# sakarias88/racer-tracer

Measured on AMD Instinct MI355X. Metric: Msamples/s (W*H*spp/s) at 1920x1080, higher is better.
Workload: dtype f64; 1 GPU; cornell_box.yml 1920x1080 1024spp max_depth 20; strip_rows=8, parallelism=image rows interleaved over 1 GPU(s)

## Files before the change

### racer-tracer_amd/csrc/rt_pool_coop.h

```cpp
#pragma once
#include "rt_pool_groups.h"
#include "rt_pool_lds.h"
#include "rt_primary_bounds.h"

namespace RT_KNS {

__device__ __forceinline__ int lane_rank(uint64_t mask) {
    return (int)__builtin_amdgcn_mbcnt_hi((uint32_t)(mask >> 32), __builtin_amdgcn_mbcnt_lo((uint32_t)mask, 0u));
}

__device__ __forceinline__ void post_request(SphereSlot *slot, const ScatterPrefix &P, uint32_t base) {
    __hip_atomic_store(&slot->b, P.b, __ATOMIC_RELAXED, __HIP_MEMORY_SCOPE_WAVEFRONT);
    __hip_atomic_store(&slot->y, P.y, __ATOMIC_RELAXED, __HIP_MEMORY_SCOPE_WAVEFRONT);
    __hip_atomic_store(&slot->x, P.x, __ATOMIC_RELAXED, __HIP_MEMORY_SCOPE_WAVEFRONT);
    __hip_atomic_store(&slot->w, P.w, __ATOMIC_RELAXED, __HIP_MEMORY_SCOPE_WAVEFRONT);
    __hip_atomic_store(&slot->z, P.z, __ATOMIC_RELAXED, __HIP_MEMORY_SCOPE_WAVEFRONT);
    __hip_atomic_store(&slot->base, base, __ATOMIC_RELAXED, __HIP_MEMORY_SCOPE_WAVEFRONT);
}
__device__ __forceinline__ void move_masked(const d3 &p, uint64_t mask, d3 &v) {
    uint64_t saved;
    asm volatile("s_and_saveexec_b64 %[saved], %[mask]\n\t"
                 "v_mov_b64 %[x], %[px]\n\t"
                 "v_mov_b64 %[y], %[py]\n\t"
                 "v_mov_b64 %[z], %[pz]\n\t"
                 "s_mov_b64 exec, %[saved]"
                 : [x] "+v"(v.x), [y] "+v"(v.y), [z] "+v"(v.z), [saved] "=&s"(saved)
                 : [mask] "s"(mask), [px] "v"(p.x), [py] "v"(p.y), [pz] "v"(p.z)
                 : "scc");
}
__device__ __forceinline__ void increment_masked(uint32_t &v, uint64_t mask) {
    asm("v_addc_co_u32 %[v], vcc, 0, %[v], %[mask]" : [v] "+v"(v) : [mask] "s"(mask) : "vcc");
}
static_assert(sizeof(TraceArgs) % alignof(rtdev::PrimaryRects) == 0, "no padding between the kernel's two arguments");
__device__ __forceinline__ const RT_CONSTANT rtdev::PrimaryRects *primary_rects_here() {
    return (const RT_CONSTANT rtdev::PrimaryRects *)((const RT_CONSTANT unsigned char *)kernargs_here() + sizeof(TraceArgs));
}
__device__ __forceinline__ uint32_t request_count(uint64_t pending) {
    uint32_t n = (uint32_t)__builtin_popcountll(pending);
    asm("" : "+s"(n));
    return n;
}

static_assert(rtdev::RT_PRIMARY_RECTS <= 32, "a rect mask is one 32-bit word");
template <bool PAIRS>
__device__ __forceinline__ void closest_hit_rects(const Prim *table, const d3 &o, const d3 &d, const d3 &inv_d, double &best_t, int &best,
                                                  uint32_t rect_mask = ~0u) {
    auto test_plane = [&](auto axis, const Prim &P, int i) {
#ifndef RT_EXACT_DIV
        rect_closest_update<decltype(axis)::value>(P.p[0], P.p[1], P.p[2], P.p[3], P.p[4], o, d, inv_d, 0.001, best_t, best, i);
        return;
#endif
        double t;
        if (rect_t<true>(decltype(axis)::value, P.p[0], P.p[1], P.p[2], P.p[3], P.p[4], o, d, inv_d, 0.001, best_t, t)) {
            best_t = t;
            best = i;
        }
    };
    const Prim *rec = table;
    int i = 0;
    auto group = [&](auto axis, int end) {
        if (PAIRS) {
            for (; i + 1 < end; i += 2, rec += 2) {
                const Prim pa = load_prim_uniform(rec, 0), pb = load_prim_uniform(rec, 1);
                test_plane(axis, pa, i);
                test_plane(axis, pb, i + 1);
            }
            if (i < end) {
                test_plane(axis, load_prim_uniform(rec, 0), i);
                ++i;
                ++rec;
            }
        } else {
            const int n = end - i;
            if (n > 0 && n < 32 && ((rect_mask >> (i & 31)) & ((1u << n) - 1u)) == 0u) {
                i = end;
                rec = reinterpret_cast<const Prim *>(reinterpret_cast<const unsigned char *>(rec) + (uint32_t)n * (uint32_t)sizeof(Prim));
            }
            for (; i < end; ++i, ++rec)
                if ((rect_mask >> (i & 31)) & 1u) test_plane(axis, load_prim_uniform(rec, 0), i);
        }
    };
    const RT_CONSTANT TraceArgs *KB = kernargs_here();
    const int end_xy = KB->rect_end[0], end_xz = KB->rect_end[1], end_yz = KB->rect_end[2];
    group(std::integral_constant<int, 2>(), end_xy);
    group(std::integral_constant<int, 1>(), end_xz);
    group(std::integral_constant<int, 0>(), end_yz);
}

template <int MAX_ROUNDS>
__device__ __forceinline__ uint64_t coop_random_in_unit_sphere(uint64_t pending, uint32_t pixel, uint32_t sample, uint32_t seg,
                                                           uint32_t &base, uint32_t k0, uint32_t k1, int lane,
                                                           SphereSlot *slot, d3 &result) {
    uint64_t have = 0;
    const ScatterPrefix own = scatter_prefix(pixel, sample, seg, k0, k1);
    auto one_round = [&](int round) {
        const bool FIRST = round == 0;
        const uint32_t n = request_count(pending);
        if (!FIRST && n < 8u) return false;
        const int lg = rt_groups::group_lg(n);
        d3 cand;
        uint64_t take;
        if (lg == 0) {
            const d3 p = sphere_candidate(philox_from_prefix(own, base, k0, k1));
            cand = p;
            take = pending;
            const uint64_t inside = ballot(len2(p) < 1.0);
            have |= pending & inside;
            pending &= ~inside;
            if (__builtin_amdgcn_inverse_ballot_w64(pending)) base += 1u;
        } else {
            const rt_groups::GroupMasks groups = rt_groups::group_masks((uint32_t)lg);
            const bool need = __builtin_amdgcn_inverse_ballot_w64(pending);
            const int rank = lane_rank(pending);
            if (need) post_request(slot + rank, own, base);
            const int j = lane >> lg;
            const int c = lane & ((1 << lg) - 1);
            const bool serving = (uint32_t)j < n;
            SphereSlot *const served = slot + (serving ? j : 0);
            const ScatterPrefix r = {served->b, served->y, served->x, served->w, served->z};
            const uint32_t i = served->base + (uint32_t)c;
            const d3 p = sphere_candidate(philox_from_prefix(r, i, k0, k1));
            const uint64_t accepted = ballot(serving) & ballot(len2(p) < 1.0);
            asm volatile("" ::: "memory");
            if (__builtin_amdgcn_inverse_ballot_w64(rt_groups::lowest_in_groups(accepted, groups))) {
                double *const answer = reinterpret_cast<double *>(served);
                answer[0] = p.x;
                answer[1] = p.y;
                answer[2] = p.z;
            }
            asm volatile("" ::: "memory");
            const int first = need ? (rank << lg) : 0;
            const uint64_t got = pending & ballot(((accepted >> first) & groups.width) != 0);
            const double *const answer = reinterpret_cast<const double *>(slot + (need ? rank : 0));
            cand = mk(answer[0], answer[1], answer[2]);
            take = got;
            have |= got;
            pending &= ~got;
            if (__builtin_amdgcn_inverse_ballot_w64(pending)) base += 1u << lg;
        }
        if (FIRST) {
            result = cand;
        } else {
            move_masked(cand, take, result);
        }
        return true;
    };
    if constexpr (MAX_ROUNDS == 2) {
#pragma unroll
// ... 100 lines not shown
```

### racer-tracer_amd/csrc/rt_scene_create.hip

```cpp
#include <hip/hip_runtime.h>
#include <stdint.h>
#include <string.h>
#include <memory>
#include <mutex>
#include <string>
#include <vector>
#include "rt_scene.h"

using rtapi::DevBuf;
using rtapi::fail;

namespace {
struct CachedSet {
    int device;
    rtapi::RenderBuffers buf;
};
std::mutex g_cache_mutex;
std::vector<CachedSet> g_cache;
const size_t kCachedSetsPerDevice = 2;

void render_cache_put(RtScene *s) {
    if (s->buf.complete()) {
        std::lock_guard<std::mutex> lock(g_cache_mutex);
        size_t held = 0;
        for (const CachedSet &c : g_cache) held += c.device == s->device;
        if (held < kCachedSetsPerDevice) {
            g_cache.push_back(CachedSet{s->device, s->buf});
            s->buf = rtapi::RenderBuffers();
            return;
        }
    }
    s->buf.free_all(s->device);
}
bool render_cache_take(RtScene *s) {
    std::lock_guard<std::mutex> lock(g_cache_mutex);
    int best = -1;
    for (size_t i = 0; i < g_cache.size(); ++i)
        if (g_cache[i].device == s->device && (best < 0 || g_cache[i].buf.partial.count > g_cache[(size_t)best].buf.partial.count))
            best = (int)i;
    if (best < 0) return false;
    s->buf = g_cache[(size_t)best].buf;
    g_cache.erase(g_cache.begin() + best);
    return true;
}

#define RT_FAST_LAUNCHER(member, name, ret, params) name,
#define RT_EXACT_LAUNCHER(member, name, ret, params) name##_exact,
const rtapi::Launchers kFastLaunchers = {RT_LAUNCHER_LIST(RT_FAST_LAUNCHER)};
const rtapi::Launchers kExactLaunchers = {RT_LAUNCHER_LIST(RT_EXACT_LAUNCHER)};
#undef RT_FAST_LAUNCHER
#undef RT_EXACT_LAUNCHER

template <class T> int upload(DevBuf<T> &buf, const std::vector<T> &host) {
    RT_HIP(buf.alloc(host.size()));
    if (!host.empty()) RT_HIP(hipMemcpy(buf.ptr, host.data(), host.size() * sizeof(T), hipMemcpyHostToDevice));
    return RT_OK;
}

int upload_images(const RtSceneDesc *d, RtScene *s, std::vector<rtdev::Image> &images) {
    images.assign((size_t)d->n_images, rtdev::Image());
    s->image_pixels.assign((size_t)d->n_images, nullptr);
    for (int i = 0; i < d->n_images; ++i) {
        size_t bytes = (size_t)d->images[i].width * (size_t)d->images[i].height * 4;
        RT_HIP(hipMalloc((void **)&s->image_pixels[(size_t)i], bytes));
        RT_HIP(hipMemcpy(s->image_pixels[(size_t)i], d->images[i].rgba, bytes, hipMemcpyHostToDevice));
        images[(size_t)i].rgba = s->image_pixels[(size_t)i];
        images[(size_t)i].width = d->images[i].width;
        images[(size_t)i].height = d->images[i].height;
    }
    return RT_OK;
}

rtdev::BvhBuild choose_bvh(const RtSceneDesc *d, const RtScene *s) {
    using rtapi::kBvhLdsBytes;
    auto blocks_with = [&](const rtdev::BvhBuild &b) {
        const size_t bytes = b.nodes.size() * sizeof(rtdev::BvhNode);
        const size_t dyn = rtdev::pool_lds_layout(true, s->textured, d->n_primitives, d->n_textures, bytes <= kBvhLdsBytes ? (int)b.nodes.size() : 0,
                                                  d->n_perlins > 0 && s->perlin_identity, false, s->has_moving).bytes;
        return s->kernels->pool_blocks_per_cu(s->prims_class, s->textured, s->specular, 1, dyn);
    };
    const bool surely_large = d->n_primitives > 2048;
    rtdev::BvhBuild bvh = rtdev::build_bvh(d->primitives, d->n_primitives, 4, surely_large);
    int max_leaf = 0;
#ifdef RT_DEVELOPER_KNOBS
    if (const char *k = getenv("RT_BVH_LEAF")) max_leaf = atoi(k);
#endif
    if (max_leaf > 0) {
        bvh = rtdev::build_bvh(d->primitives, d->n_primitives, max_leaf);
    } else if (bvh.nodes.size() * sizeof(rtdev::BvhNode) <= kBvhLdsBytes) {
// ... 45 lines not shown
        s->pool_dyn_lds = dyn_lds(false);
        s->pool_dyn_lds_lens = dyn_lds(true);
        s->pool_static_lds = s->kernels->pool_static_lds(s->prims_class, s->textured, s->specular, s->use_bvh);
        if (s->pool_static_lds < 0) return fail(RT_ERR_HIP, "hipFuncGetAttributes of the trace kernel failed");
        s->pool_blocks_per_cu = s->kernels->pool_blocks_per_cu(s->prims_class, s->textured, s->specular, s->use_bvh, s->pool_dyn_lds);
        s->pool_blocks_per_cu_lens = s->kernels->pool_blocks_per_cu(s->prims_class, s->textured, s->specular, s->use_bvh, s->pool_dyn_lds_lens);
    }
#ifdef RT_DEVELOPER_KNOBS
    if (const char *k = getenv("RT_POOL_BLOCKS_PER_CU"))
        if (atoi(k) > 0) s->pool_blocks_per_cu = s->pool_blocks_per_cu_lens = atoi(k);
#endif
    return RT_OK;
}

int acquire_render_buffers(RtScene *s) {
    rtapi::RenderBuffers &b = s->buf;
    if (!render_cache_take(s)) {
        RT_HIP(b.segments.alloc(rtdev::RT_STAT_SLOTS));
        RT_HIP(hipStreamCreateWithFlags(&b.stream, hipStreamNonBlocking));
        RT_HIP(hipEventCreate(&b.ev_begin));
        RT_HIP(hipEventCreate(&b.ev_traced));
        RT_HIP(hipEventCreate(&b.ev_resolved));
        RT_HIP(hipHostMalloc((void **)&b.host_flags, (rtdev::RT_MAX_REGIONS + 1) * sizeof(unsigned int),
                             hipHostMallocPortable | hipHostMallocMapped | hipHostMallocCoherent));
        memset(b.host_flags, 0, (rtdev::RT_MAX_REGIONS + 1) * sizeof(unsigned int));
        RT_HIP(hipStreamCreateWithFlags(&b.stream_ctl, hipStreamNonBlocking));
    }
    RT_HIP(hipMemsetAsync(b.segments.ptr, 0, rtdev::RT_STAT_SLOTS * sizeof(unsigned long long), b.stream));
    return RT_OK;
}

int scene_create(const RtSceneDesc *d, int device, const RtSceneOptions *options, RtScene **out) {
    if (!out) return fail(RT_ERR_INVALID_ARGUMENT, "out is NULL");
    *out = nullptr;
    int rc = rtapi::validate_desc(d);
    if (rc != RT_OK) return rc;
    RtSceneOptions opt;
    if ((rc = rtapi::check_options(options, opt)) != RT_OK) return rc;
    int n_dev = rt_device_count();
    if (n_dev <= 0) return fail(RT_ERR_NO_DEVICE, "no HIP device is visible to this process");
    if (device < 0 || device >= n_dev) return fail(RT_ERR_INVALID_ARGUMENT, "device index out of range");
    RT_HIP(hipSetDevice(device));

    RtScene *s = new RtScene();
    std::unique_ptr<RtScene, void (*)(RtScene *)> half_built(s, rt_scene_destroy);
    s->device = device;
    s->exact = opt.arithmetic == RT_ARITH_REFERENCE;
    s->gather_staged = opt.gather == RT_GATHER_STAGED;
    s->use_v1 = opt.kernel == RT_KERNEL_V1;

    std::vector<rtdev::Prim> prims = rtapi::pack_prims(d);
    s->radiance_bound = rtapi::scene_radiance_bound(d);
    const std::vector<rtdev::Perlin> perlins = rtapi::pack_perlins(d, s->perlin_identity);
    const rtapi::Selection sel = rtapi::select_variant(d);
    s->prims_class = sel.prims_class;
    s->textured = sel.textured;
    s->specular = sel.specular;
    s->has_moving = sel.has_moving;
    rtapi::scene_bounds(d, s->box_mn, s->box_mx);
    s->use_bvh = d->n_primitives > rtapi::kBvhThreshold;
    if (opt.closest_hit != RT_HIT_AUTO) s->use_bvh = opt.closest_hit == RT_HIT_BVH && d->n_primitives > 0;
    if (s->radiance_bound == 0.0 && !s->use_v1 && (s->use_bvh || s->prims_class == 2)) s->exact = true;
    s->kernels = s->exact ? &kExactLaunchers : &kFastLaunchers;
    if (!s->use_bvh && (size_t)d->n_primitives * sizeof(rtdev::Prim) > rtapi::kLinearTableBytes)
        return fail(RT_ERR_UNSUPPORTED, "RT_HIT_LINEAR: the primitive table does not fit in LDS");

    std::vector<int32_t> order((size_t)d->n_primitives);
    for (size_t j = 0; j < order.size(); ++j) order[j] = (int32_t)j;
    rtdev::BvhBuild bvh;
    rtapi::LeafTable leaves;
    if (s->use_bvh) {
        bvh = choose_bvh(d, s);
        order.assign(bvh.prim_index.begin(), bvh.prim_index.end());
        std::vector<rtdev::Prim> ordered(prims.size());
        for (size_t j = 0; j < bvh.prim_index.size(); ++j) ordered[j] = prims[(size_t)bvh.prim_index[j]];
        prims.swap(ordered);
        leaves = rtapi::leaf_geometry(prims);
    } else {
        const rtapi::LinearGroups groups = rtapi::group_linear_table(prims, order);
        for (int g = 0; g < 3; ++g) s->rect_end[g] = groups.rect_end[g];
        s->sphere_end = groups.sphere_end;
        s->box_end = groups.box_end;
        const int n_rects = groups.rect_end[2];
        if (n_rects == d->n_primitives && n_rects <= rtdev::RT_PRIMARY_RECTS)
            for (int j = 0; j < n_rects; ++j) {
                const rtdev::Prim &q = prims[(size_t)j];
                s->primary_rect_geo.push_back(rtdev::RectGeo{j < groups.rect_end[0] ? 2 : (j < groups.rect_end[1] ? 1 : 0), q.p[0], q.p[1], q.p[2], q.p[3], q.p[4]});
            }
    }
    const rtapi::LightTables lights = rtapi::light_tables(d, order, rtapi::kMaxLights);

    std::vector<rtdev::Image> images;
    if ((rc = upload_images(d, s, images)) != RT_OK) return rc;
    const std::vector<rtdev::Texture> textures = rtapi::pack_textures(d, images);
    if (s->use_bvh && (rc = upload_bvh(s, bvh, leaves)) != RT_OK) return rc;
    if ((rc = rtapi::build_light_list(s, lights)) != RT_OK) return rc;
    s->light_facts = rtapi::light_facts(d);
    s->table_order = order;
    s->pick_weights.assign(lights.lights.size(), lights.lights.empty() ? 0.0 : 1.0 / (double)lights.lights.size());
    if ((rc = upload(s->prims, prims)) != RT_OK) return rc;
    if ((rc = upload(s->textures, textures)) != RT_OK) return rc;
    if ((rc = upload(s->images, images)) != RT_OK) return rc;
    if ((rc = upload(s->perlins, perlins)) != RT_OK) return rc;
    s->n_prims = d->n_primitives;
    s->n_materials = d->n_materials;
    s->n_textures = d->n_textures;
    s->n_images = d->n_images;
    s->n_perlins = d->n_perlins;
    s->bg.kind = d->background.kind;
    for (int k = 0; k < 3; ++k) {
        s->bg.top[k] = d->background.top[k];
        s->bg.bottom[k] = d->background.bottom[k];
    }
    if ((rc = size_pool(s)) != RT_OK) return rc;
    if ((rc = acquire_render_buffers(s)) != RT_OK) return rc;
    *out = half_built.release();
    return RT_OK;
}

}

extern "C" {

void rt_scene_destroy(RtScene *s) {
    if (!s) return;
    (void)hipSetDevice(s->device);
    if (s->buf.stream) (void)hipStreamSynchronize(s->buf.stream);
    if (s->buf.stream_ctl) (void)hipStreamSynchronize(s->buf.stream_ctl);
    for (uint8_t *p : s->image_pixels)
        if (p) (void)hipFree(p);
    s->prims.release();
    s->textures.release();
    s->images.release();
    s->perlins.release();
    s->bvh_nodes.release();
    s->bvh_nodes_ordered.release();
    s->bvh_prim_index.release();
    s->leaf_geo.release();
    s->nee_slot.release();
    s->nee_prim.release();
    s->nee_pick.release();
    if (rtapi::guarded("rt_scene_destroy", [&] { render_cache_put(s); return RT_OK; }) != RT_OK) s->buf.free_all(s->device);
    delete s;
}

void rt_release_cached_buffers(void) {
    (void)rtapi::guarded("rt_release_cached_buffers", [] {
        std::vector<CachedSet> all;
        {
            std::lock_guard<std::mutex> lock(g_cache_mutex);
            all.swap(g_cache);
        }
        for (CachedSet &c : all) c.buf.free_all(c.device);
        return RT_OK;
    });
}

int rt_scene_create(const RtSceneDesc *d, int device, RtScene **out) {
    return rtapi::guarded("rt_scene_create", [&] { return scene_create(d, device, nullptr, out); });
}

int rt_scene_create_ex(const RtSceneDesc *d, int device, const RtSceneOptions *options, RtScene **out) {
    return rtapi::guarded("rt_scene_create_ex", [&] { return scene_create(d, device, options, out); });
}

int rtdev_scene_classify(const RtSceneDesc *d, int32_t out[4]) {
// ... 37 lines not shown
```

### racer-tracer_amd/csrc/rt_trace_common.h

```cpp
#pragma once
#include <hip/hip_runtime.h>
#include <stdint.h>
#include "rt_device_types.h"
#include "rt_bvh_slab.h"
#include "../../include/rt_abi.h"
#include "../../include/rt_rng.h"

#ifdef RT_EXACT_DIV
#define RT_KNS rtdev_exact
#define RT_LAUNCHER(name) name##_exact
#else
#define RT_KNS rtdev_fast
#define RT_LAUNCHER(name) name
#endif

namespace RT_KNS {
using namespace rtdev;

#define RT_CONSTANT __attribute__((address_space(4)))
__device__ __forceinline__ Prim load_prim_uniform(const Prim *table, int i) {
    Prim p;
    __builtin_memcpy(&p, (const RT_CONSTANT Prim *)(table + i), sizeof(Prim));
    return p;
}
// ... 152 lines not shown
    const uint32_t d_hi = __builtin_amdgcn_alignbit(0x400u, w, 12);
    return __longlong_as_double((long long)(((unsigned long long)d_hi << 32) | d_lo)) - 3.0;
}
__device__ __forceinline__ double sym42(uint32_t w, uint32_t t_at_10) {
    return sym42_bits((w << 20) | t_at_10, w);
}
__device__ __forceinline__ d3 sphere_candidate(const u4 &b) {
    return mk(sym42_bits(__builtin_amdgcn_alignbit(b.a, b.d << 22, 12), b.a), sym42(b.b, b.d & 0x000FFC00u),
              sym42(b.c, (b.d >> 10) & 0x000FFC00u));
}

struct PathRng {
    uint32_t pixel, sample, k0, k1;
    __device__ __forceinline__ u4 block(uint32_t segment, uint32_t purpose, uint32_t blk) const {
        return philox4x32(pixel, sample, (segment << 8) | purpose, blk, k0, k1);
    }
};

__device__ __forceinline__ d3 random_in_unit_sphere(const PathRng &rng, uint32_t segment) {
    for (uint32_t i = 0;; ++i) {
        d3 p = sphere_candidate(rng.block(segment, RT_RNG_SCATTER, i));
        if (len2(p) >= 1.0) continue;
        return p;
    }
}

struct Hit {
    d3 point, normal;
    double u, v;
    bool front;
    bool uv_approx;
};

__device__ __forceinline__ void set_face_normal(Hit &h, d3 dir, d3 outward) {
    h.front = dot(dir, outward) < 0.0;
    const uint32_t flip = h.front ? 0u : 0x80000000u;
    auto with_sign = [flip](double x) {
        return __longlong_as_double((long long)((unsigned long long)__double_as_longlong(x) ^ ((unsigned long long)flip << 32)));
    };
    h.normal = mk(with_sign(outward.x), with_sign(outward.y), with_sign(outward.z));
}

__device__ __forceinline__ void set_face_normal_axis(Hit &h, d3 dir, int axis) {
#ifdef RT_EXACT_DIV
    set_face_normal(h, dir, mk(axis == 0 ? 1.0 : 0.0, axis == 1 ? 1.0 : 0.0, axis == 2 ? 1.0 : 0.0));
#else
    auto against = [](double dk) {
        const uint32_t hi = 0xBFF00000u ^ ((uint32_t)((unsigned long long)__double_as_longlong(dk) >> 32) & 0x80000000u);
        return __longlong_as_double((long long)((unsigned long long)hi << 32));
    };
    h.normal = mk(axis == 0 ? against(dir.x) : 0.0, axis == 1 ? against(dir.y) : 0.0, axis == 2 ? against(dir.z) : 0.0);
    h.front = h.normal.x + h.normal.y + h.normal.z > 0.0;
#endif
}

__device__ __forceinline__ d3 rot_fwd(d3 a, double s, double c) {
    return mk(c * a.x - s * a.z, a.y, s * a.x + c * a.z);
}
__device__ __forceinline__ d3 rot_back(d3 a, double s, double c) {
    return mk(c * a.x + s * a.z, a.y, -s * a.x + c * a.z);
}

template <bool EARLY_OUT>
__device__ __forceinline__ bool rect_t(int axis, double a0, double a1, double b0, double b1, double k,
                                       d3 o, d3 d, d3 inv_d, double t_min, double t_max, double &t_out) {
    int ia = axis == 0 ? 1 : 0;
    int ib = axis == 2 ? 1 : 2;
    const double t = div_by(k - comp(o, axis), comp(d, axis), comp(inv_d, axis));
    if (EARLY_OUT) {
        if (t < t_min || t > t_max) return false;
        const double a = comp(o, ia) + t * comp(d, ia);
        const double b = comp(o, ib) + t * comp(d, ib);
        if (a < a0 || a > a1 || b < b0 || b > b1) return false;
        t_out = t;
        return true;
    }
    const double a = comp(o, ia) + t * comp(d, ia);
    const double b = comp(o, ib) + t * comp(d, ib);
    const bool miss = (t < t_min) | (t > t_max) | (a < a0) | (a > a1) | (b < b0) | (b > b1);
    t_out = t;
    return !miss;
}

template <int AXIS>
__device__ __forceinline__ void rect_closest_update(double a0, double a1, double b0, double b1, double k, d3 o, d3 d, d3 inv_d,
                                                    double t_min, double &best_t, int &best, int i) {
    constexpr int IA = AXIS == 0 ? 1 : 0, IB = AXIS == 2 ? 1 : 2;
    double t, a, b;
    unsigned long long saved;
    asm volatile("v_add_f64 %[t], %[k], -%[oc]\n\t"
                 "v_mul_f64 %[t], %[inv], %[t]\n\t"
                 "s_mov_b64 %[saved], exec\n\t"
                 "v_cmpx_ngt_f64 %[tmin], %[t]\n\t"
                 "v_cmpx_ngt_f64 %[t], %[bt]\n\t"
                 "s_cbranch_execz 1f\n\t"
                 "v_fma_f64 %[a], %[da], %[t], %[oa]\n\t"
                 "v_fma_f64 %[b], %[db], %[t], %[ob]\n\t"
                 "v_cmpx_ngt_f64 %[a0], %[a]\n\t"
                 "v_cmpx_nlt_f64 %[a1], %[a]\n\t"
                 "v_cmpx_ngt_f64 %[b0], %[b]\n\t"
                 "v_cmpx_nlt_f64 %[b1], %[b]\n\t"
                 "v_mov_b64 %[bt], %[t]\n\t"
                 "v_mov_b32 %[best], %[i]\n"
                 "1:\n\t"
                 "s_mov_b64 exec, %[saved]"
                 : [t] "=&v"(t), [a] "=&v"(a), [b] "=&v"(b), [saved] "=&s"(saved), [bt] "+v"(best_t), [best] "+v"(best)
                 : [k] "s"(k), [oc] "v"(comp(o, AXIS)), [inv] "v"(comp(inv_d, AXIS)), [tmin] "s"(t_min), [da] "v"(comp(d, IA)),
                   [oa] "v"(comp(o, IA)), [db] "v"(comp(d, IB)), [ob] "v"(comp(o, IB)), [a0] "s"(a0), [a1] "s"(a1), [b0] "s"(b0),
                   [b1] "s"(b1), [i] "s"(i)
                 : "vcc");
}

__device__ __forceinline__ void box_side(const double *p, int s, int &axis, double &a0, double &a1,
                                         double &b0, double &b1, double &k) {
    axis = 2 - (s >> 1);
    if (axis == 2) { a0 = p[0]; a1 = p[3]; b0 = p[1]; b1 = p[4]; k = (s & 1) ? p[2] : p[5]; }
    else if (axis == 1) { a0 = p[0]; a1 = p[3]; b0 = p[2]; b1 = p[5]; k = (s & 1) ? p[1] : p[4]; }
    else { a0 = p[1]; a1 = p[4]; b0 = p[2]; b1 = p[5]; k = (s & 1) ? p[0] : p[3]; }
}

__device__ __forceinline__ bool sphere_t(d3 center, double radius2, d3 o, d3 d, double inv_a, double t_min, double t_max,
                                         double &t_out) {
    const d3 oc = o - center;
    const double a = len2(d);
    const double half_b = dot(oc, d);
    const double c = len2(oc) - radius2;
    const double disc = half_b * half_b - a * c;
    if (disc < 0.0) return false;
    const double sqrtd = sqrt_fast(disc);
    double root = div_by(-half_b - sqrtd, a, inv_a);
    if (root < t_min || t_max < root) {
        root = div_by(-half_b + sqrtd, a, inv_a);
        if (root < t_min || t_max < root) return false;
    }
    t_out = root;
    return true;
}

__device__ __forceinline__ bool box_slab_t(const double *p, d3 o, d3 d, d3 inv_d, double t_min, double t_max, double &t_out,
                                           int &side) {
    const double x_mn = div_by(p[0] - o.x, d.x, inv_d.x), x_mx = div_by(p[3] - o.x, d.x, inv_d.x);
    const double y_mn = div_by(p[1] - o.y, d.y, inv_d.y), y_mx = div_by(p[4] - o.y, d.y, inv_d.y);
    const double z_mn = div_by(p[2] - o.z, d.z, inv_d.z), z_mx = div_by(p[5] - o.z, d.z, inv_d.z);
    const double x_near = fmin(x_mn, x_mx), x_far = fmax(x_mn, x_mx);
    const double y_near = fmin(y_mn, y_mx), y_far = fmax(y_mn, y_mx);
    const double z_near = fmin(z_mn, z_mx), z_far = fmax(z_mn, z_mx);
    const double t_enter = fmax(fmax(x_near, y_near), z_near);
    const double t_exit = fmin(fmin(x_far, y_far), z_far);
    const bool entry = t_enter >= t_min;
    const double t = entry ? t_enter : t_exit;
    const int side_in = t_enter == z_near ? 0 : (t_enter == y_near ? 2 : 4);
    const int side_out = t_exit == z_far ? 0 : (t_exit == y_far ? 2 : 4);
    side = entry ? side_in : side_out;
    t_out = t;
    return t_enter <= t_exit && t >= t_min && t <= t_max;
}

template <int PRIMS>
__device__ __forceinline__ bool prim_t(const Prim &P, d3 o, d3 d, d3 inv_d, double inv_a, double time, double t_min,
                                       double t_max, double &t_out, int &aux) {
    aux = 0;
    if (PRIMS == PRIMS_RECTS) {
        int kind = P.kind;
        if (kind == RT_PRIM_XY_RECT) return rect_t<true>(2, P.p[0], P.p[1], P.p[2], P.p[3], P.p[4], o, d, inv_d, t_min, t_max, t_out);
        if (kind == RT_PRIM_XZ_RECT) return rect_t<true>(1, P.p[0], P.p[1], P.p[2], P.p[3], P.p[4], o, d, inv_d, t_min, t_max, t_out);
        return rect_t<true>(0, P.p[0], P.p[1], P.p[2], P.p[3], P.p[4], o, d, inv_d, t_min, t_max, t_out);
    }
    if (PRIMS == PRIMS_ANY) {
        if (P.flags & RT_PRIM_HAS_TRANSLATE) o = o - ld3(P.tr);
        if (P.flags & RT_PRIM_HAS_ROTATE_Y) {
            o = rot_fwd(o, P.rot_sin, P.rot_cos);
            d = rot_fwd(d, P.rot_sin, P.rot_cos);
            inv_d.x = rcp_f64(d.x);
            inv_d.z = rcp_f64(d.z);
        }
    }
    switch (PRIMS == PRIMS_SPHERES ? (int)RT_PRIM_SPHERE : P.kind) {
    case RT_PRIM_MOVING_SPHERE:
    case RT_PRIM_SPHERE: {
        d3 center = ld3(P.p);
        if (PRIMS == PRIMS_ANY && P.kind == RT_PRIM_MOVING_SPHERE)
            center = center + ((time - P.rot_sin) * P.rot_cos) * ld3(P.tr);
        return sphere_t(center, P.radius2, o, d, inv_a, t_min, t_max, t_out);
    }
    case RT_PRIM_XY_RECT: return rect_t<true>(2, P.p[0], P.p[1], P.p[2], P.p[3], P.p[4], o, d, inv_d, t_min, t_max, t_out);
    case RT_PRIM_XZ_RECT: return rect_t<true>(1, P.p[0], P.p[1], P.p[2], P.p[3], P.p[4], o, d, inv_d, t_min, t_max, t_out);
    case RT_PRIM_YZ_RECT: return rect_t<true>(0, P.p[0], P.p[1], P.p[2], P.p[3], P.p[4], o, d, inv_d, t_min, t_max, t_out);
    default: {
#ifndef RT_EXACT_DIV
        return box_slab_t(P.p, o, d, inv_d, t_min, t_max, t_out, aux);
#endif
        bool any = false;
        double closest = t_max;
// ... 409 lines not shown
```

### racer-tracer_amd/csrc/rt_trace_pool_kernel.hip

```cpp
#include <cstddef>
#include <type_traits>
#include "rt_trace_common.h"
#include "rt_primary_bounds.h"
#include "rt_variant_dispatch.h"
#include "rt_pool_profile.h"
#include "rt_pool_lds.h"
#include "rt_pool_coop.h"
#include "rt_pool_deliver.h"

#ifndef RT_OCC_TEX
#define RT_OCC_TEX 4
#endif
#ifndef RT_OCC_TEX_BVH
#define RT_OCC_TEX_BVH 4
#endif
#ifndef RT_OCC_TEX_ANY
#define RT_OCC_TEX_ANY 4
#endif
#ifndef RT_OCC_SPEC
#define RT_OCC_SPEC 5
#endif
#ifndef RT_OCC_ANY
#define RT_OCC_ANY 5
#endif
// ... 492 lines not shown
                        d = mk(signed_like(0u), signed_like(1u), signed_like(2u));
                        T = mk(1.0, 1.0, 1.0);
                        seg = 0;
                        asm volatile("; hand_out_end");
                    }
                    alive_m |= taking;
                }
                RT_REGION(2);
                if (alive_m == 0) break;
                uint64_t ended_m = 0;
                const uint64_t hit_m = alive_m & ~waiting_m;
                int kind;
                asm volatile("" : "=v"(kind));
                if (__builtin_amdgcn_inverse_ballot_w64(hit_m)) {
                    const Prim &P = lds_prims[best];
                    const Material &M = P.mat;
                    kind = M.kind;
                    RT_REGION(8);
                    T = T * ld3(M.color);
                    RT_REGION(9);
                    cand_base = 0;
#ifndef RT_EXACT_DIV
                    {
                        const int axis = P.kind == RT_PRIM_XY_RECT ? 2 : (P.kind == RT_PRIM_XZ_RECT ? 1 : 0);
                        auto against = [](double dk, bool on_axis) {
                            uint32_t lo = 0u;
                            asm volatile("" : "+v"(lo));
                            const uint32_t hi = on_axis ? 0xBFF00000u ^ ((uint32_t)((unsigned long long)__double_as_longlong(dk) >> 32) & 0x80000000u) : 0u;
                            return __longlong_as_double((long long)((unsigned long long)hi << 32 | lo));
                        };
                        const uint64_t xy_m = ballot(axis == 2), xz_m = ballot(axis == 1);
                        d = mk(against(d.x, __builtin_amdgcn_inverse_ballot_w64(~(xy_m | xz_m))), against(d.y, __builtin_amdgcn_inverse_ballot_w64(xz_m)),
                               against(d.z, __builtin_amdgcn_inverse_ballot_w64(xy_m)));
                    }
#else
                    {
                        Hit h;
                        set_face_normal_axis(h, d, P.kind == RT_PRIM_XY_RECT ? 2 : (P.kind == RT_PRIM_XZ_RECT ? 1 : 0));
                        d = h.normal;
                    }
#endif
                }
                asm volatile("" : "+v"(kind));
                const uint64_t light_m = hit_m & ballot(kind == RT_MAT_DIFFUSE_LIGHT);
                ended_m |= light_m;
                waiting_m |= hit_m & ~light_m;
                RT_REGION(4);
                d3 sph = mk(0.0, 0.0, 0.0);
                const uint64_t finish_m = coop_random_in_unit_sphere<2>(waiting_m, rng.pixel, rng.sample, seg, cand_base, A.seed_lo, A.seed_hi, lane,
                                                                        L.scratch.sphere, sph);
                waiting_m &= ~finish_m;
                RT_REGION(5);
                if (__builtin_amdgcn_inverse_ballot_w64(finish_m)) {
                    const d3 dir = d + unit_fast(sph);
                    const uint64_t near_zero = ballot(fabs(dir.x) < 1e-8) & ballot(fabs(dir.y) < 1e-8) & ballot(fabs(dir.z) < 1e-8);
#ifndef RT_EXACT_DIV
                    d = dir;
                    if (near_zero != 0) {
                        asm volatile("; near_zero (keeps the compiler from turning the branch back into selects)");
                        if ((near_zero >> lane) & 1ull) {
                            const d3 u = unit_fast(sph);
                            d = mk(rint(-u.x) + 0.0, rint(-u.y) + 0.0, rint(-u.z) + 0.0);
                        }
                    }
#else
                    const d3 normal = d;
                    d = dir;
                    if (near_zero != 0) {
                        asm volatile("; near_zero (keeps the compiler from turning the branch back into selects)");
                        if ((near_zero >> lane) & 1ull) d = normal;
                    }
#endif
                }
                increment_masked(seg, finish_m);
                const uint64_t deep_m = finish_m & ballot((int)seg >= A.max_depth);
                ended_m |= deep_m;
                const uint64_t shooting = finish_m & ~deep_m;
                RT_LANES(__popcll(shooting), next >= total);
                asm volatile("" : "=v"(best));
                if (__builtin_amdgcn_inverse_ballot_w64(shooting)) {
                    double best_t = __builtin_inf();
                    best = -1;
                    ++n_segments;
                    closest_hit_rects<true>(A.prims, o, d, rcp3(d), best_t, best);
                    asm volatile("; hit_point_begin" : "+v"(best_t));
                    o = ray_at(o, best_t, d);
                    asm volatile("; hit_point_end" : "+v"(o.x), "+v"(o.y), "+v"(o.z));
                    RT_REGION(3);
                }
                const uint64_t miss_m = shooting & ballot(best < 0);
                uint64_t adding_m = ended_m;
                ended_m |= miss_m;
                if (kernargs_here()->bg_black == 0) {
                    adding_m = ended_m;
                    const RT_CONSTANT TraceArgs *K = kernargs_here();
                    const uint64_t sky_m = K->bg.kind == RT_BG_SKY ? miss_m : 0ull;
                    if (__builtin_amdgcn_inverse_ballot_w64(miss_m & ~sky_m)) {
                        T.x = T.x * K->bg.top[0];
                        T.y = T.y * K->bg.top[1];
                        T.z = T.z * K->bg.top[2];
                    }
                    if (__builtin_amdgcn_inverse_ballot_w64(sky_m)) {
                        const double t = 0.5 * (unit_fast(d).y + 1.0);
                        T = T * ((1.0 - t) * ld3(K->bg.top) + t * ld3(K->bg.bottom));
                    }
                }
                if (__builtin_amdgcn_inverse_ballot_w64(adding_m)) {
                    atomicAdd(&L.sum[spix][0], T.x);
                    atomicAdd(&L.sum[spix][1], T.y);
                    atomicAdd(&L.sum[spix][2], T.z);
                }
                alive_m &= ~ended_m;
                RT_REGION(6);
            }
        } else
        for (;;) {
        while (next >= batch_due) {
            prepare_batch(batches_done++);
            batch_due = batches_done >= n_batches ? ~0u : (batches_done < (uint32_t)NBUF ? 0u : (batches_done - (uint32_t)(NBUF - 1)) << 6);
        }
        RT_REGION(1);
        if (next < total) {
            const uint64_t idle = ~alive_m;
            const uint32_t w = next + (uint32_t)lane_rank(idle);
            const uint32_t ready = NBUF == 2 ? total : min(total, batches_done << 6);
            next = min(next + (uint32_t)__popcll(idle), ready);
            if (OVERLAP && next >= total) state |= POOL_DRY;
            int s_off, pix_new;
            if (n_valid == 64) {
                pix_new = (int)(w & 63u);
                s_off = (int)(w >> 6);
            } else {
                s_off = (int)(w / (uint32_t)n_valid);
                pix_new = L.pix_of[w - (uint32_t)s_off * (uint32_t)n_valid];
            }
            const uint32_t pixel_new = (uint32_t)shfl_i((int)my_pixel, pix_new);
            const uint64_t taking = idle & ballot(w < ready);
            if (__builtin_amdgcn_inverse_ballot_w64(taking)) {
                spix = (int)(state & CUR) | pix_new;
                rng.pixel = pixel_new;
                rng.sample = (uint32_t)(smp0 + s_off);
                const RT_CONSTANT TraceArgs *K = kernargs_here();
                const int buf = (int)((w >> 6) & (uint32_t)(NBUF - 1)), slot = (int)(w & 63u);
                const double v = L.v[buf][slot];
                const d3 co = ld3(K->cam.origin);
                o = co;
                if (OVERLAP) d = (ld3(L.ulc) + L.u[pix_new] * ld3(K->cam.horizontal)) - v * ld3(K->cam.vertical) - co;
                else d = ld3(L.base[pix_new]) - v * ld3(K->cam.vertical) - co;
                const double lr = K->cam.lens_radius;
                if (lr != 0.0) {
                    const d3 offset = ld3(K->cam.right) * lens[buf][slot][0] + ld3(K->cam.up) * lens[buf][slot][1];
                    o = co + offset;
                    d = d - offset;
                }
                if (PRIMS == PRIMS_ANY && ray_times != nullptr) ray_time = ray_times[buf][slot];
                T = mk(1.0, 1.0, 1.0);
                seg = 0;
                ++n_started;
            }
            alive_m |= taking;
        }
        RT_REGION(2);
        if (!OVERLAP && alive_m == 0) break;
        uint64_t ended_m = 0;
        uint64_t scattered_m = 0;
        uint64_t finish_m = 0;
        const uint64_t tracing = alive_m & ~waiting_m;
// ... 372 lines not shown
```

Baseline: 44630 Msamples/s.

## Skip the farther plane of facing rect pairs using per-lane near-plane selection

At scene build, consecutive axis-aligned rects with identical extents but different offsets (like opposite Cornell box walls) are marked as facing pairs, and byte offsets are stored in an unused Prim field. In the closest-hit loop, each lane uses the sign of its ray direction to pick the nearer plane of the pair from the LDS copy of the table and tests only that one. The second plane is skipped for the whole wave when every lane's other-plane t is below t_min. This adds LDS loads, a ballot and a per-lane k and index, so when the wave disagrees both planes are tested plus the extra overhead.

```diff
diff --git a/racer-tracer_amd/csrc/rt_pool_coop.h b/racer-tracer_amd/csrc/rt_pool_coop.h
--- a/racer-tracer_amd/csrc/rt_pool_coop.h
+++ b/racer-tracer_amd/csrc/rt_pool_coop.h
@@ -2,8 +2,12 @@
 #include "rt_pool_groups.h"
 #include "rt_pool_lds.h"
 #include "rt_primary_bounds.h"
+#include "rt_rect_pairs.h"
 
 namespace RT_KNS {
+
+static_assert(sizeof(Prim) == rt_pairs::kRecordBytes && offsetof(Prim, p) + 4 * sizeof(double) == rt_pairs::kOffsetOfK,
+              "rt_rect_pairs.h addresses k in the table's bytes");
 
 __device__ __forceinline__ int lane_rank(uint64_t mask) {
     return (int)__builtin_amdgcn_mbcnt_hi((uint32_t)(mask >> 32), __builtin_amdgcn_mbcnt_lo((uint32_t)mask, 0u));
@@ -44,7 +48,7 @@
 static_assert(rtdev::RT_PRIMARY_RECTS <= 32, "a rect mask is one 32-bit word");
 template <bool PAIRS>
 __device__ __forceinline__ void closest_hit_rects(const Prim *table, const d3 &o, const d3 &d, const d3 &inv_d, double &best_t, int &best,
-                                                  uint32_t rect_mask = ~0u) {
+                                                  uint32_t rect_mask = ~0u, const Prim *lds_table = nullptr) {
     auto test_plane = [&](auto axis, const Prim &P, int i) {
 #ifndef RT_EXACT_DIV
         rect_closest_update<decltype(axis)::value>(P.p[0], P.p[1], P.p[2], P.p[3], P.p[4], o, d, inv_d, 0.001, best_t, best, i);
@@ -62,8 +66,42 @@
         if (PAIRS) {
             for (; i + 1 < end; i += 2, rec += 2) {
                 const Prim pa = load_prim_uniform(rec, 0), pb = load_prim_uniform(rec, 1);
+#ifndef RT_EXACT_DIV
+                constexpr int AXIS = decltype(axis)::value;
+                const RT_CONSTANT uint32_t *words = (const RT_CONSTANT uint32_t *)rec;
+                uint32_t larger = words[(rt_pairs::kOffsetOfK + 12u) / 4u], step = words[(rt_pairs::kRecordBytes + rt_pairs::kOffsetOfK + 12u) / 4u];
+                asm volatile("; pair requested" : "+s"(larger), "+s"(step) : "s"(pa.p[0]), "s"(pa.p[1]), "s"(pa.p[2]), "s"(pa.p[3]));
+                double k_first;
+                int i_first;
+                uint32_t second = 1u;
+                auto plain = [&] {
+                    k_first = pa.p[4];
+                    i_first = i;
+                    asm volatile("; both records" : "+v"(k_first), "+v"(i_first));
+                };
+                if (larger != 0u) {
+                    using lds_bytes = const __attribute__((address_space(3))) unsigned char *;
+                    const uint32_t k_of_larger = (uint32_t)(uintptr_t)(lds_bytes)reinterpret_cast<const unsigned char *>(lds_table) + larger;
+                    const uint32_t sel = rt_pairs::selected(k_of_larger, step, rt_pairs::sign_mask(comp(d, AXIS)));
+                    const double k_other = *(const __attribute__((address_space(3))) double *)(uintptr_t)rt_pairs::partner(k_of_larger, step, sel);
+                    k_first = *(const __attribute__((address_space(3))) double *)(uintptr_t)sel;
+                    i_first = *(const __attribute__((address_space(3))) int *)(uintptr_t)(sel + 8u);
+                    asm volatile("; facing pair" : "+v"(k_first), "+v"(i_first));
+                    if (ballot(!rt_pairs::settled(rt_pairs::t_of_plane(k_other, comp(o, AXIS), comp(inv_d, AXIS)))) == 0) {
+                        second = 0u;
+                    } else {
+                        plain();
+                    }
+                } else {
+                    plain();
+                }
+                rect_closest_update<AXIS, true>(pa.p[0], pa.p[1], pa.p[2], pa.p[3], k_first, o, d, inv_d, 0.001, best_t, best, i_first);
+                asm("" : "+s"(second));
+                if (second != 0u) test_plane(axis, pb, i + 1);
+#else
                 test_plane(axis, pa, i);
                 test_plane(axis, pb, i + 1);
+#endif
             }
             if (i < end) {
                 test_plane(axis, load_prim_uniform(rec, 0), i);
diff --git a/racer-tracer_amd/csrc/rt_rect_pairs.h b/racer-tracer_amd/csrc/rt_rect_pairs.h
--- /dev/null
+++ b/racer-tracer_amd/csrc/rt_rect_pairs.h
@@ -0,0 +1,63 @@
+#pragma once
+#include <stdint.h>
+#include <cmath>
+#include "rt_primary_bounds.h"
+
+#if defined(__HIPCC__)
+#define RT_PAIRS_FN __host__ __device__ inline
+#else
+#define RT_PAIRS_FN inline
+#endif
+
+namespace rt_pairs {
+
+RT_PAIRS_FN uint64_t bits_of(double v) {
+    uint64_t b;
+    __builtin_memcpy(&b, &v, sizeof b);
+    return b;
+}
+
+inline bool facing_pair(const rtdev::RectGeo &a, const rtdev::RectGeo &b) {
+    return a.axis == b.axis && bits_of(a.a0) == bits_of(b.a0) && bits_of(a.a1) == bits_of(b.a1) && bits_of(a.b0) == bits_of(b.b0) &&
+           bits_of(a.b1) == bits_of(b.b1) && std::isfinite(a.k) && std::isfinite(b.k) && a.k != b.k;
+}
+
+enum : uint32_t { kRecordBytes = 192, kOffsetOfK = 32 };
+struct Fields {
+    uint64_t first, second;
+};
+inline Fields mark_facing(int i, double k_a, double k_b) {
+    const uint32_t larger = (uint32_t)(k_a > k_b ? i : i + 1) * kRecordBytes + kOffsetOfK;
+    const uint32_t step = k_a > k_b ? (uint32_t)kRecordBytes : 0u - (uint32_t)kRecordBytes;
+    return Fields{(uint64_t)(uint32_t)i | (uint64_t)larger << 32, (uint64_t)(uint32_t)(i + 1) | (uint64_t)step << 32};
+}
+inline uint64_t mark_single(int i) { return (uint64_t)(uint32_t)i; }
+inline void mark_table(const rtdev::RectGeo *geo, const int32_t rect_end[3], uint64_t *field) {
+    for (int j = 0; j < rect_end[2]; ++j) field[j] = mark_single(j);
+    for (int g = 0, first = 0; g < 3; first = rect_end[g++])
+        for (int j = first; j + 1 < rect_end[g]; j += 2)
+            if (facing_pair(geo[j], geo[j + 1])) {
+                const Fields f = mark_facing(j, geo[j].k, geo[j + 1].k);
+                field[j] = f.first;
+                field[j + 1] = f.second;
+            }
+}
+RT_PAIRS_FN uint32_t larger_of(uint64_t first_bits) { return (uint32_t)(first_bits >> 32); }
+RT_PAIRS_FN uint32_t step_of(uint64_t second_bits) { return (uint32_t)(second_bits >> 32); }
+
+RT_PAIRS_FN uint32_t sign_mask(double d_c) {
+    const uint32_t hi = (uint32_t)(bits_of(d_c) >> 32);
+#if defined(__HIP_DEVICE_COMPILE__)
+    uint32_t mask;
+    asm("v_ashrrev_i32 %0, 31, %1" : "=v"(mask) : "v"(hi));
+    return mask;
+#else
+    return (uint32_t)((int32_t)hi >> 31);
+#endif
+}
+RT_PAIRS_FN uint32_t selected(uint32_t larger, uint32_t step, uint32_t sign) { return larger + (sign & step); }
+RT_PAIRS_FN uint32_t partner(uint32_t larger, uint32_t step, uint32_t sel) { return (2u * larger + step) - sel; }
+RT_PAIRS_FN double t_of_plane(double k, double o_c, double inv_c) { return (k - o_c) * inv_c; }
+RT_PAIRS_FN bool settled(double t_other) { return t_other < 0.001; }
+
+}
diff --git a/racer-tracer_amd/csrc/rt_scene_create.hip b/racer-tracer_amd/csrc/rt_scene_create.hip
--- a/racer-tracer_amd/csrc/rt_scene_create.hip
+++ b/racer-tracer_amd/csrc/rt_scene_create.hip
@@ -5,6 +5,7 @@
 #include <mutex>
 #include <string>
 #include <vector>
+#include "rt_rect_pairs.h"
 #include "rt_scene.h"
 
 using rtapi::DevBuf;
@@ -216,6 +217,16 @@
         s->sphere_end = groups.sphere_end;
         s->box_end = groups.box_end;
         const int n_rects = groups.rect_end[2];
+        {
+            std::vector<rtdev::RectGeo> geo;
+            for (int j = 0; j < n_rects; ++j) {
+                const rtdev::Prim &q = prims[(size_t)j];
+                geo.push_back(rtdev::RectGeo{j < groups.rect_end[0] ? 2 : (j < groups.rect_end[1] ? 1 : 0), q.p[0], q.p[1], q.p[2], q.p[3], q.p[4]});
+            }
+            std::vector<uint64_t> field((size_t)n_rects);
+            rt_pairs::mark_table(geo.data(), groups.rect_end, field.data());
+            for (int j = 0; j < n_rects; ++j) memcpy(&prims[(size_t)j].p[5], &field[(size_t)j], sizeof(uint64_t));
+        }
         if (n_rects == d->n_primitives && n_rects <= rtdev::RT_PRIMARY_RECTS)
             for (int j = 0; j < n_rects; ++j) {
                 const rtdev::Prim &q = prims[(size_t)j];
diff --git a/racer-tracer_amd/csrc/rt_trace_common.h b/racer-tracer_amd/csrc/rt_trace_common.h
--- a/racer-tracer_amd/csrc/rt_trace_common.h
+++ b/racer-tracer_amd/csrc/rt_trace_common.h
@@ -258,33 +258,43 @@
     return !miss;
 }
 
-template <int AXIS>
+#define RT_RECT_CLOSEST_UPDATE_TEXT                                                                                        \
+    "v_add_f64 %[t], %[k], -%[oc]\n\t"                                                                                      \
+    "v_mul_f64 %[t], %[inv], %[t]\n\t"                             \
+    "s_mov_b64 %[saved], exec\n\t"                                                                                          \
+    "v_cmpx_ngt_f64 %[tmin], %[t]\n\t"                                              \
+    "v_cmpx_ngt_f64 %[t], %[bt]\n\t"                                            \
+    "s_cbranch_execz 1f\n\t"                                 \
+    "v_fma_f64 %[a], %[da], %[t], %[oa]\n\t"                                                          \
+    "v_fma_f64 %[b], %[db], %[t], %[ob]\n\t"                                                                                \
+    "v_cmpx_ngt_f64 %[a0], %[a]\n\t"             \
+    "v_cmpx_nlt_f64 %[a1], %[a]\n\t"                                                                                        \
+    "v_cmpx_ngt_f64 %[b0], %[b]\n\t"                                                                                        \
+    "v_cmpx_nlt_f64 %[b1], %[b]\n\t"                                                                                        \
+    "v_mov_b64 %[bt], %[t]\n\t"                                              \
+    "v_mov_b32 %[best], %[i]\n"                                                                                             \
+    "1:\n\t"                                                                                                               \
+    "s_mov_b64 exec, %[saved]"
+template <int AXIS, bool K_PER_LANE = false>
 __device__ __forceinline__ void rect_closest_update(double a0, double a1, double b0, double b1, double k, d3 o, d3 d, d3 inv_d,
                                                     double t_min, double &best_t, int &best, int i) {
     constexpr int IA = AXIS == 0 ? 1 : 0, IB = AXIS == 2 ? 1 : 2;
     double t, a, b;
     unsigned long long saved;
-    asm volatile("v_add_f64 %[t], %[k], -%[oc]\n\t"
-                 "v_mul_f64 %[t], %[inv], %[t]\n\t"
-                 "s_mov_b64 %[saved], exec\n\t"
-                 "v_cmpx_ngt_f64 %[tmin], %[t]\n\t"
-                 "v_cmpx_ngt_f64 %[t], %[bt]\n\t"
-                 "s_cbranch_execz 1f\n\t"
-                 "v_fma_f64 %[a], %[da], %[t], %[oa]\n\t"
-                 "v_fma_f64 %[b], %[db], %[t], %[ob]\n\t"
-                 "v_cmpx_ngt_f64 %[a0], %[a]\n\t"
-                 "v_cmpx_nlt_f64 %[a1], %[a]\n\t"
-                 "v_cmpx_ngt_f64 %[b0], %[b]\n\t"
-                 "v_cmpx_nlt_f64 %[b1], %[b]\n\t"
-                 "v_mov_b64 %[bt], %[t]\n\t"
-                 "v_mov_b32 %[best], %[i]\n"
-                 "1:\n\t"
-                 "s_mov_b64 exec, %[saved]"
-                 : [t] "=&v"(t), [a] "=&v"(a), [b] "=&v"(b), [saved] "=&s"(saved), [bt] "+v"(best_t), [best] "+v"(best)
-                 : [k] "s"(k), [oc] "v"(comp(o, AXIS)), [inv] "v"(comp(inv_d, AXIS)), [tmin] "s"(t_min), [da] "v"(comp(d, IA)),
-                   [oa] "v"(comp(o, IA)), [db] "v"(comp(d, IB)), [ob] "v"(comp(o, IB)), [a0] "s"(a0), [a1] "s"(a1), [b0] "s"(b0),
-                   [b1] "s"(b1), [i] "s"(i)
-                 : "vcc");
+    if constexpr (K_PER_LANE)
+        asm volatile(RT_RECT_CLOSEST_UPDATE_TEXT
+                     : [t] "=&v"(t), [a] "=&v"(a), [b] "=&v"(b), [saved] "=&s"(saved), [bt] "+v"(best_t), [best] "+v"(best)
+                     : [k] "v"(k), [oc] "v"(comp(o, AXIS)), [inv] "v"(comp(inv_d, AXIS)), [tmin] "s"(t_min), [da] "v"(comp(d, IA)),
+                       [oa] "v"(comp(o, IA)), [db] "v"(comp(d, IB)), [ob] "v"(comp(o, IB)), [a0] "s"(a0), [a1] "s"(a1), [b0] "s"(b0),
+                       [b1] "s"(b1), [i] "v"(i)
+                     : "vcc");
+    else
+        asm volatile(RT_RECT_CLOSEST_UPDATE_TEXT
+                     : [t] "=&v"(t), [a] "=&v"(a), [b] "=&v"(b), [saved] "=&s"(saved), [bt] "+v"(best_t), [best] "+v"(best)
+                     : [k] "s"(k), [oc] "v"(comp(o, AXIS)), [inv] "v"(comp(inv_d, AXIS)), [tmin] "s"(t_min), [da] "v"(comp(d, IA)),
+                       [oa] "v"(comp(o, IA)), [db] "v"(comp(d, IB)), [ob] "v"(comp(o, IB)), [a0] "s"(a0), [a1] "s"(a1), [b0] "s"(b0),
+                       [b1] "s"(b1), [i] "s"(i)
+                     : "vcc");
 }
 
 __device__ __forceinline__ void box_side(const double *p, int s, int &axis, double &a0, double &a1,
diff --git a/racer-tracer_amd/csrc/rt_trace_pool_kernel.hip b/racer-tracer_amd/csrc/rt_trace_pool_kernel.hip
--- a/racer-tracer_amd/csrc/rt_trace_pool_kernel.hip
+++ b/racer-tracer_amd/csrc/rt_trace_pool_kernel.hip
@@ -598,7 +598,7 @@
                     double best_t = __builtin_inf();
                     best = -1;
                     ++n_segments;
-                    closest_hit_rects<true>(A.prims, o, d, rcp3(d), best_t, best);
+                    closest_hit_rects<true>(A.prims, o, d, rcp3(d), best_t, best, ~0u, lds_prims);
                     asm volatile("; hit_point_begin" : "+v"(best_t));
                     o = ray_at(o, best_t, d);
                     asm volatile("; hit_point_end" : "+v"(o.x), "+v"(o.y), "+v"(o.z));
```

Measured after the change: 45140 Msamples/s (median of 6 runs). 1.01x the previous value.
